# gongaa/Feedback-GNN

Measured on NVIDIA B200. Metric: decoded frames/sec (BP->GNN->BP, [[1270,28]]), higher is better.
Workload: dtype f32

## Files before the change

### feedback-gnn_b200/csrc/fbgnn_gbp_tc.cuh

```cuda
#ifndef FBGNN_GBP_TC_CUH
#define FBGNN_GBP_TC_CUH

#include "fbgnn_kernels.cuh"

namespace fbgnn {
namespace tc {

__device__ __forceinline__ uint32_t smem_u32(const void *p) { return (uint32_t)__cvta_generic_to_shared(p); }

__device__ __forceinline__ void tmem_alloc(uint32_t *slot, uint32_t ncols) {
    asm volatile("tcgen05.alloc.cta_group::1.sync.aligned.shared::cta.b32 [%0], %1;" :: "r"(smem_u32(slot)), "r"(ncols) : "memory");
    asm volatile("tcgen05.relinquish_alloc_permit.cta_group::1.sync.aligned;" ::: "memory");
}
__device__ __forceinline__ void tmem_dealloc(uint32_t taddr, uint32_t ncols) {
    asm volatile("tcgen05.dealloc.cta_group::1.sync.aligned.b32 %0, %1;" :: "r"(taddr), "r"(ncols) : "memory");
}
__device__ __forceinline__ void tc_fence_before() { asm volatile("tcgen05.fence::before_thread_sync;" ::: "memory"); }
__device__ __forceinline__ void tc_fence_after() { asm volatile("tcgen05.fence::after_thread_sync;" ::: "memory"); }
__device__ __forceinline__ void fence_async_smem() { asm volatile("fence.proxy.async.shared::cta;" ::: "memory"); }
__device__ __forceinline__ void tmem_wait_st() { asm volatile("tcgen05.wait::st.sync.aligned;" ::: "memory"); }
__device__ __forceinline__ void tmem_wait_ld() { asm volatile("tcgen05.wait::ld.sync.aligned;" ::: "memory"); }

__device__ __forceinline__ void tmem_st8(uint32_t taddr, const uint32_t v[8]) {
    asm volatile("tcgen05.st.sync.aligned.32x32b.x8.b32 [%0], {%1, %2, %3, %4, %5, %6, %7, %8};"
                 :: "r"(taddr), "r"(v[0]), "r"(v[1]), "r"(v[2]), "r"(v[3]), "r"(v[4]), "r"(v[5]), "r"(v[6]), "r"(v[7]) : "memory");
}
__device__ __forceinline__ void tmem_ld8(uint32_t taddr, float v[8]) {
    uint32_t r[8];
    asm volatile("tcgen05.ld.sync.aligned.32x32b.x8.b32 {%0, %1, %2, %3, %4, %5, %6, %7}, [%8];"
                 : "=r"(r[0]), "=r"(r[1]), "=r"(r[2]), "=r"(r[3]), "=r"(r[4]), "=r"(r[5]), "=r"(r[6]), "=r"(r[7]) : "r"(taddr) : "memory");
    asm volatile("tcgen05.wait::ld.sync.aligned;" ::: "memory");
#pragma unroll
    for (int q = 0; q < 8; q++) v[q] = __uint_as_float(r[q]);
}

__device__ __forceinline__ void umma_tf32_ts(uint32_t d_tmem, uint32_t a_tmem, uint64_t b_desc, uint32_t idesc, uint32_t accumulate) {
    asm volatile("{\n\t.reg .pred p;\n\tsetp.ne.b32 p, %4, 0;\n\t"
                 "tcgen05.mma.cta_group::1.kind::tf32 [%0], [%1], %2, %3, p;\n\t}"
                 :: "r"(d_tmem), "r"(a_tmem), "l"(b_desc), "r"(idesc), "r"(accumulate) : "memory");
}
__device__ __forceinline__ void umma_commit(uint32_t bar) {
    asm volatile("tcgen05.commit.cta_group::1.mbarrier::arrive::one.shared::cluster.b64 [%0];" :: "r"(bar) : "memory");
}
__device__ __forceinline__ void mbar_init(uint64_t *bar, uint32_t count) {
    asm volatile("mbarrier.init.shared::cta.b64 [%0], %1;" :: "r"(smem_u32(bar)), "r"(count) : "memory");
    asm volatile("fence.mbarrier_init.release.cluster;" ::: "memory");
}
__device__ __forceinline__ void mbar_wait(uint32_t bar, uint32_t parity) {
    uint32_t ok;
    do {
        asm volatile("{\n\t.reg .pred p;\n\tmbarrier.try_wait.parity.shared::cta.b64 p, [%1], %2;\n\tselp.b32 %0, 1, 0, p;\n\t}"
                     : "=r"(ok) : "r"(bar), "r"(parity) : "memory");
    } while (!ok);
}

__host__ __device__ inline int b_tile_offset(int n, int k, int kpad) {
    return (n >> 3) * (kpad / 4) * 32 + (k >> 2) * 32 + (n & 7) * 4 + (k & 3);
}
__device__ __forceinline__ uint64_t b_desc(uint32_t saddr, int kpad) {
    const uint64_t lbo = 128 >> 4, sbo = (uint64_t)((kpad / 4) * 128) >> 4;
    return (uint64_t)((saddr & 0x3FFFF) >> 4) | (lbo << 16) | (sbo << 32) | (1ull << 46);
}
__host__ __device__ inline uint32_t idesc_tf32(int npad) {
    return (1u << 4) | (2u << 7) | (2u << 10) | ((uint32_t)(npad >> 3) << 17) | ((128u >> 4) << 24);
}
__host__ __device__ inline float tf32_hi(float x) {
#ifdef __CUDA_ARCH__
    return __uint_as_float((__float_as_uint(x) + 0x1000u) & 0xffffe000u);
#else
    uint32_t u; memcpy(&u, &x, 4); u = (u + 0x1000u) & 0xffffe000u; float r; memcpy(&r, &u, 4); return r;
#endif
}

constexpr int t(int k, int n) { return 2 * k * n; }
struct VnW {
    static constexpr int B1X = 0, B1Z = B1X + t(24, 48);
    static constexpr int W2X = B1Z + t(24, 48), W2Z = W2X + t(40, 32);
    static constexpr int W3AB = W2Z + t(40, 32);
    static constexpr int W3C = W3AB + t(40, 48);
    static constexpr int W4 = W3C + t(24, 48);
    static constexpr int W5 = W4 + t(40, 32);
    static constexpr int BIAS = W5 + t(24, 80);
    static constexpr int total = BIAS + 180;
};
struct CnW {
    static constexpr int B1 = 0, W2 = B1 + t(24, 48);
    static constexpr int W3A = W2 + t(40, 32);
    static constexpr int W3B = W3A + t(24, 48);
    static constexpr int W4 = W3B + t(24, 48);
    static constexpr int W5 = W4 + t(40, 32);
    static constexpr int BIAS = W5 + t(24, 48);
    static constexpr int total = BIAS + 120;
};

struct Grp {
    uint32_t tmem;
    uint32_t lane_base;
    uint32_t bar;
    uint32_t phase;
    int gid;
    bool leader;
};

__device__ __forceinline__ void grp_sync(int gid) { asm volatile("bar.sync %0, 128;" :: "r"(gid + 1) : "memory"); }

template <int KPAD>
__device__ __forceinline__ void store_a(const Grp &g, int col_hi, int col_lo, const float *a) {
    __syncwarp();
#pragma unroll
    for (int k0 = 0; k0 < KPAD; k0 += 8) {
        uint32_t hi[8], lo[8];
#pragma unroll
        for (int q = 0; q < 8; q++) {
            const float h = tf32_hi(a[k0 + q]);
            hi[q] = __float_as_uint(h);
            lo[q] = __float_as_uint(a[k0 + q] - h);
        }
        tmem_st8(g.lane_base + col_hi + k0, hi);
        tmem_st8(g.lane_base + col_lo + k0, lo);
    }
}

__device__ __forceinline__ void gemm(Grp &g, int col_ahi, int col_alo, int kpad, int col_d, uint32_t b_saddr, int npad,
                                     bool accumulate) {
    __syncwarp();
    tmem_wait_st();
    tmem_wait_ld();
    tc_fence_before();
    grp_sync(g.gid);
    if (g.leader) {
        tc_fence_after();
        const uint32_t idesc = idesc_tf32(npad);
        const uint32_t bl = b_saddr + (uint32_t)(npad * kpad * 4);
        for (int s = 0; s < kpad / 8; s++) {
            const uint64_t dh = b_desc(b_saddr + s * 256, kpad), dl = b_desc(bl + s * 256, kpad);
            umma_tf32_ts(g.tmem + col_d, g.tmem + col_ahi + s * 8, dh, idesc, (accumulate || s > 0) ? 1u : 0u);
            umma_tf32_ts(g.tmem + col_d, g.tmem + col_alo + s * 8, dh, idesc, 1u);
            umma_tf32_ts(g.tmem + col_d, g.tmem + col_ahi + s * 8, dl, idesc, 1u);
        }
        umma_commit(g.bar);
    }
    mbar_wait(g.bar, g.phase);
    g.phase ^= 1u;
    tc_fence_after();
    __syncwarp();
}

template <typename MATH, typename SENDER>
__device__ __forceinline__ int recv_tc(const Grp &g, int col_base, const float *__restrict__ b1, int e0, int e1,
                                       const float *__restrict__ rows, int row_stride, uint32_t *codes, int cstride,
                                       SENDER sender) {
    constexpr int JB = 8, H = 40;
    gbp_stage_codes(codes, cstride, e0, e1, sender);
    auto code_at = [&](int e) -> uint32_t { return (e - e0 < GBP_CODE_CAP) ? codes[(e - e0) * cstride] : sender(e); };
    int ssum = 0;
    uint32_t c0 = 0;
    float4 nx0 = make_float4(0.0f, 0.0f, 0.0f, 0.0f), nx1 = nx0;
    if (e0 < e1) {
        c0 = code_at(e0);
        const float *pf = rows + (int64_t)(c0 >> 1) * row_stride;
        nx0 = *reinterpret_cast<const float4 *>(pf); nx1 = *reinterpret_cast<const float4 *>(pf + 4);
    }
#pragma unroll 1
    for (int j = 0; j < H; j += JB) {
        float bs[JB], hs[JB];
        __syncwarp();
        tmem_ld8(g.lane_base + col_base + j, bs);
        const float4 ba = *reinterpret_cast<const float4 *>(b1 + j), bb = *reinterpret_cast<const float4 *>(b1 + j + 4);
        bs[0] += ba.x; bs[1] += ba.y; bs[2] += ba.z; bs[3] += ba.w; bs[4] += bb.x; bs[5] += bb.y; bs[6] += bb.z; bs[7] += bb.w;
#pragma unroll
        for (int q = 0; q < JB; q++) hs[q] = 0.0f;
        uint32_t cc = c0;
#pragma unroll 1
        for (int e = e0; e < e1; e++) {
            const float pq[JB] = {nx0.x, nx0.y, nx0.z, nx0.w, nx1.x, nx1.y, nx1.z, nx1.w};
            const bool neg = (cc & 1u) != 0;
            if (e + 1 < e1) {
                cc = code_at(e + 1);
                const float *pf = rows + (int64_t)(cc >> 1) * row_stride + j;
                nx0 = *reinterpret_cast<const float4 *>(pf); nx1 = *reinterpret_cast<const float4 *>(pf + 4);
            }
            if (j == 0) ssum += neg ? -1 : 1;
#pragma unroll
            for (int q = 0; q < JB; q++) {
                float t = MATH::tanh(pq[q] + bs[q]);
                hs[q] += neg ? -t : t;
            }
        }
        if (j + JB < H && e0 < e1) {
            const float *pf = rows + (int64_t)(c0 >> 1) * row_stride + j + JB;
            nx0 = *reinterpret_cast<const float4 *>(pf); nx1 = *reinterpret_cast<const float4 *>(pf + 4);
        }
        uint32_t hi[JB], lo[JB];
#pragma unroll
        for (int q = 0; q < JB; q++) {
            const float h = tf32_hi(hs[q]);
            hi[q] = __float_as_uint(h);
            lo[q] = __float_as_uint(hs[q] - h);
        }
        __syncwarp();
        tmem_st8(g.lane_base + j, hi);
        tmem_st8(g.lane_base + H + j, lo);
    }
    return ssum;
}

__device__ __forceinline__ void bulk_g2s(uint32_t dst_saddr, const void *src, uint32_t bytes, uint32_t bar) {
    asm volatile("cp.async.bulk.shared::cluster.global.mbarrier::complete_tx::bytes [%0], [%1], %2, [%3];"
                 :: "r"(dst_saddr), "l"(src), "r"(bytes), "r"(bar) : "memory");
}
__device__ __forceinline__ void mbar_expect_tx(uint32_t bar, uint32_t bytes) {
    asm volatile("mbarrier.arrive.expect_tx.shared::cta.b64 _, [%0], %1;" :: "r"(bar), "r"(bytes) : "memory");
}

__device__ __forceinline__ Grp cta_setup(float *sm, const float *__restrict__ wsrc, int nfloats, uint64_t *bars, uint32_t *tslot) {
    __shared__ uint64_t load_bar;
    if (threadIdx.x < 32) tmem_alloc(tslot, 256);
    if (threadIdx.x == 32) {
        mbar_init(&bars[0], 1); mbar_init(&bars[1], 1); mbar_init(&load_bar, 1);
        fence_async_smem();
        const uint32_t bytes = (uint32_t)nfloats * 4u, bar = smem_u32(&load_bar), dst = smem_u32(sm);
        mbar_expect_tx(bar, bytes);
        constexpr uint32_t CHUNK = 32768;
        for (uint32_t off = 0; off < bytes; off += CHUNK)
            bulk_g2s(dst + off, reinterpret_cast<const char *>(wsrc) + off, min(CHUNK, bytes - off), bar);
    }
    tc_fence_before();
    __syncthreads();
    tc_fence_after();
    mbar_wait(smem_u32(&load_bar), 0);
    Grp g;
    g.gid = threadIdx.x >> 7;
    const int t = threadIdx.x & 127;
    g.tmem = *tslot + (uint32_t)(g.gid * 128);
    g.lane_base = g.tmem + ((uint32_t)((t >> 5) * 32) << 16);
    g.bar = smem_u32(&bars[g.gid]);
    g.phase = 0;
    g.leader = t == 0;
    return g;
}

__device__ __forceinline__ void cta_teardown(const uint32_t *tslot) {
    tmem_wait_ld();
    tmem_wait_st();
    tc_fence_before();
    __syncthreads();
    if (threadIdx.x < 32) tmem_dealloc(*tslot, 256);
}

template <typename MATH>
__global__ void __launch_bounds__(256, 2) k_gbp_vn_tc(const GbpArgs a, const float *__restrict__ wtc) {
    constexpr int D = 20, H = 40, M = 20;
    extern __shared__ __align__(128) float sm[];
    __shared__ uint64_t bars[2];
    __shared__ uint32_t tslot;
    Grp g = cta_setup(sm, wtc, VnW::total, bars, &tslot);
    const uint32_t sbase = smem_u32(sm);
    const float *bias = sm + VnW::BIAS;
    uint32_t *codes = reinterpret_cast<uint32_t *>(sm + VnW::total) + threadIdx.x;
    const int n = a.X.n, mt = a.X.m + a.Z.m, t = threadIdx.x & 127;
    const int64_t total = a.B * n, ntiles = (total + 127) / 128;
    for (int64_t tile = (int64_t)blockIdx.x * 2 + g.gid; tile < ntiles; tile += (int64_t)gridDim.x * 2) {
        const int64_t it = tile * 128 + t;
        const bool valid = it < total;
        const int64_t b = valid ? it / n : 0;
        const int v = valid ? (int)(it - b * n) : 0;
        float own[24], mm[2 * M];
#pragma unroll
        for (int k = 0; k < 24; k++) own[k] = 0.0f;
        if (valid) {
#pragma unroll
            for (int k = 0; k < D; k += 4) {
                const float4 v4 = *reinterpret_cast<const float4 *>(a.h_vn + it * D + k);
                own[k] = v4.x; own[k + 1] = v4.y; own[k + 2] = v4.z; own[k + 3] = v4.w;
            }
        }
#pragma unroll 1
        for (int side = 0; side < 2; side++) {
            const SideDev &S = side ? a.Z : a.X;
            const float *pf_b = a.pfc + (b * mt + (side ? a.X.m : 0)) * H;
            const uint8_t *sy = side ? a.sz + b * a.Z.m : a.sx + b * a.X.m;
            const idx_t *vn_cn = S.vn_cn;
            const int e0 = valid ? S.vn_ptr[v] : 0, e1 = valid ? S.vn_ptr[v + 1] : 0;
            store_a<24>(g, 0, 24, own);
            gemm(g, 0, 24, 24, 80, sbase + 4 * (side ? VnW::B1Z : VnW::B1X), 48, false);
            const int ssum = recv_tc<MATH>(g, 80, bias + side * H, e0, e1, pf_b, H, codes, 256,
                                           [&](int e) { const uint32_t c = vn_cn[e]; return (c << 1) | (sy[c] != 0 ? 1u : 0u); });
            gemm(g, 0, 40, 40, 80, sbase + 4 * (side ? VnW::W2Z : VnW::W2X), 32, false);
            const float fs = (float)ssum, dg = (float)(e1 - e0);
            const float *b2 = bias + 2 * H + side * M;
#pragma unroll
            for (int c0 = 0; c0 < 24; c0 += 8) {
                float d[8];
                tmem_ld8(g.lane_base + 80 + c0, d);
#pragma unroll
                for (int q = 0; q < 8; q++) {
                    if (c0 + q < M) {
                        float r = d[q] + fs * b2[c0 + q];
                        if (a.reduce == 0 && e1 > e0) r = r / dg;
                        if (side == 0) mm[c0 + q] = r;
                        else mm[M + c0 + q] = r;
                    }
                }
            }
        }
        store_a<40>(g, 0, 40, mm);
        gemm(g, 0, 40, 40, 80, sbase + 4 * VnW::W3AB, 48, false);
        store_a<24>(g, 0, 24, own);
        gemm(g, 0, 24, 24, 80, sbase + 4 * VnW::W3C, 48, true);
        float hid[H];
        const float *b3 = bias + 2 * H + 2 * M;
#pragma unroll
        for (int c0 = 0; c0 < H; c0 += 8) {
            float d[8];
            tmem_ld8(g.lane_base + 80 + c0, d);
#pragma unroll
            for (int q = 0; q < 8; q++) hid[c0 + q] = MATH::tanh(d[q] + b3[c0 + q]);
        }
        store_a<40>(g, 0, 40, hid);
        gemm(g, 0, 40, 40, 80, sbase + 4 * VnW::W4, 32, false);
        float out[24];
        const float *b4 = b3 + H;
#pragma unroll
        for (int c0 = 0; c0 < 24; c0 += 8) {
            float d[8];
            tmem_ld8(g.lane_base + 80 + c0, d);
#pragma unroll
            for (int q = 0; q < 8; q++) out[c0 + q] = (c0 + q < D) ? d[q] + b4[c0 + q] : 0.0f;
        }
        if (valid) {
#pragma unroll
            for (int k = 0; k < D; k += 4)
                *reinterpret_cast<float4 *>(a.h_vn + it * D + k) = make_float4(out[k], out[k + 1], out[k + 2], out[k + 3]);
        }
        store_a<24>(g, 80, 104, out);
        gemm(g, 80, 104, 24, 0, sbase + 4 * VnW::W5, 80, false);
#pragma unroll 1
        for (int c0 = 0; c0 < 2 * H; c0 += 8) {
            float d[8];
            __syncwarp();
            tmem_ld8(g.lane_base + c0, d);
            if (valid) {
                float *dst = a.pfv + it * 2 * H + c0;
                *reinterpret_cast<float4 *>(dst) = make_float4(d[0], d[1], d[2], d[3]);
                *reinterpret_cast<float4 *>(dst + 4) = make_float4(d[4], d[5], d[6], d[7]);
            }
        }
    }
    cta_teardown(&tslot);
}

template <typename MATH>
__global__ void __launch_bounds__(256, 2) k_gbp_cn_tc(const GbpArgs a, const float *__restrict__ wtc, int side) {
    constexpr int D = 20, H = 40, M = 20;
    extern __shared__ __align__(128) float sm[];
    __shared__ uint64_t bars[2];
    __shared__ uint32_t tslot;
    Grp g = cta_setup(sm, wtc, CnW::total, bars, &tslot);
    const uint32_t sbase = smem_u32(sm);
    const float *bias = sm + CnW::BIAS;
    uint32_t *codes = reinterpret_cast<uint32_t *>(sm + CnW::total) + threadIdx.x;
    const SideDev &S = side ? a.Z : a.X;
    const int n = a.X.n, mt = a.X.m + a.Z.m, ms = S.m, coff = side ? a.X.m : 0, t = threadIdx.x & 127;
    const idx_t *cn_vn = S.cn_vn;
    float *hcs = side ? a.hcz : a.hcx;
    const uint8_t *sys = side ? a.sz : a.sx;
    const int64_t total = a.B * ms, ntiles = (total + 127) / 128;
    for (int64_t tile = (int64_t)blockIdx.x * 2 + g.gid; tile < ntiles; tile += (int64_t)gridDim.x * 2) {
        const int64_t it = tile * 128 + t;
        const bool valid = it < total;
        const int64_t b = valid ? it / ms : 0;
        const int c = valid ? (int)(it - b * ms) : 0;
        float own[24], in[24];
#pragma unroll
        for (int k = 0; k < 24; k++) { own[k] = 0.0f; in[k] = 0.0f; }
        int e0 = 0, e1 = 0;
        if (valid) {
#pragma unroll
            for (int k = 0; k < D; k += 4) {
                const float4 v4 = *reinterpret_cast<const float4 *>(hcs + it * D + k);
                own[k] = v4.x; own[k + 1] = v4.y; own[k + 2] = v4.z; own[k + 3] = v4.w;
            }
            e0 = S.cn_ptr[c]; e1 = S.cn_ptr[c + 1];
            if (!a.zero_logits) {
                const float lgv = a.lg[b * mt + coff + c];
                in[M] = sys[it] ? -lgv : lgv;
            }
        }
        const float *pf_b = a.pfv + b * n * 2 * H + (side ? H : 0);
        store_a<24>(g, 0, 24, own);
        gemm(g, 0, 24, 24, 80, sbase + 4 * CnW::B1, 48, false);
        recv_tc<MATH>(g, 80, bias, e0, e1, pf_b, 2 * H, codes, 256, [&](int e) { return (uint32_t)cn_vn[e] << 1; });
        gemm(g, 0, 40, 40, 80, sbase + 4 * CnW::W2, 32, false);
        const float dg = (float)(e1 - e0);
        const float *b2 = bias + H;
#pragma unroll
        for (int c0 = 0; c0 < 24; c0 += 8) {
            float d[8];
            tmem_ld8(g.lane_base + 80 + c0, d);
#pragma unroll
            for (int q = 0; q < 8; q++) {
                if (c0 + q < M) {
                    float r = d[q] + dg * b2[c0 + q];
                    if (a.reduce == 0 && e1 > e0) r = r / dg;
                    in[c0 + q] = r;
                }
            }
        }
        store_a<24>(g, 0, 24, in);
        gemm(g, 0, 24, 24, 80, sbase + 4 * CnW::W3A, 48, false);
        store_a<24>(g, 0, 24, own);
        gemm(g, 0, 24, 24, 80, sbase + 4 * CnW::W3B, 48, true);
        float hid[H];
        const float *b3 = bias + H + M;
#pragma unroll
        for (int c0 = 0; c0 < H; c0 += 8) {
            float d[8];
            tmem_ld8(g.lane_base + 80 + c0, d);
#pragma unroll
            for (int q = 0; q < 8; q++) hid[c0 + q] = MATH::tanh(d[q] + b3[c0 + q]);
        }
        store_a<40>(g, 0, 40, hid);
        gemm(g, 0, 40, 40, 80, sbase + 4 * CnW::W4, 32, false);
        float out[24];
        const float *b4 = b3 + H;
#pragma unroll
        for (int c0 = 0; c0 < 24; c0 += 8) {
            float d[8];
            tmem_ld8(g.lane_base + 80 + c0, d);
#pragma unroll
            for (int q = 0; q < 8; q++) out[c0 + q] = (c0 + q < D) ? d[q] + b4[c0 + q] : 0.0f;
        }
        if (valid) {
#pragma unroll
            for (int k = 0; k < D; k += 4)
                *reinterpret_cast<float4 *>(hcs + it * D + k) = make_float4(out[k], out[k + 1], out[k + 2], out[k + 3]);
        }
        store_a<24>(g, 80, 104, out);
        gemm(g, 80, 104, 24, 0, sbase + 4 * CnW::W5, 48, false);
#pragma unroll 1
        for (int c0 = 0; c0 < H; c0 += 8) {
            float d[8];
            __syncwarp();
            tmem_ld8(g.lane_base + c0, d);
            if (valid) {
                float *dst = a.pfc + (b * mt + coff + c) * H + c0;
                *reinterpret_cast<float4 *>(dst) = make_float4(d[0], d[1], d[2], d[3]);
                *reinterpret_cast<float4 *>(dst + 4) = make_float4(d[4], d[5], d[6], d[7]);
            }
        }
    }
    cta_teardown(&tslot);
}

}
}

#endif
```

### feedback-gnn_b200/csrc/fbgnn_gnn_tc.cuh

```cuda
#ifndef FBGNN_GNN_TC_CUH
#define FBGNN_GNN_TC_CUH

#include "fbgnn_gbp_tc.cuh"

namespace fbgnn {
namespace tc {

struct GnnW {
    static constexpr int H = 40, M = 20;
    static constexpr int W2X = 0, W2Z = W2X + t(40, 32);
    static constexpr int W3AB = W2Z + t(40, 32);
    static constexpr int SCALAR = W3AB + t(40, 48);
    static constexpr int total = SCALAR + GnnLayout<40, 20>::total;
};

template <int DV, typename MATH>
__device__ __forceinline__ void gnn_edges_tc(const Grp &g, const float *__restrict__ w1p, const float *__restrict__ b1,
                                             const float hc[DV], float f1, float f2, float f3) {
    constexpr int H = 40, JB = 8;
#pragma unroll 1
    for (int j0 = 0; j0 < H; j0 += JB) {
        uint32_t hi[JB], lo[JB];
#pragma unroll
        for (int q = 0; q < JB; q += 2) {
            const float4 wa = *reinterpret_cast<const float4 *>(w1p + 4 * (j0 + q));
            const float4 wb = *reinterpret_cast<const float4 *>(w1p + 4 * (j0 + q) + 4);
            float2 hs;
            if constexpr (MATH::kPaired) {
                const float2 wcn = make_float2(wa.x, wa.y);
                const float2 base = FB_FMA2(fb2s(f3), make_float2(wb.z, wb.w), FB_FMA2(fb2s(f2), make_float2(wb.x, wb.y),
                                            FB_FMA2(fb2s(f1), make_float2(wa.z, wa.w), make_float2(b1[j0 + q], b1[j0 + q + 1]))));
                hs = MATH::tanh2(FB_FMA2(fb2s(hc[0]), wcn, base));
#pragma unroll
                for (int k = 1; k < DV; k++) hs = FB_ADD2(hs, MATH::tanh2(FB_FMA2(fb2s(hc[k]), wcn, base)));
            } else {
                const float base0 = FB_FMA(f3, wb.z, FB_FMA(f2, wb.x, FB_FMA(f1, wa.z, b1[j0 + q])));
                const float base1 = FB_FMA(f3, wb.w, FB_FMA(f2, wb.y, FB_FMA(f1, wa.w, b1[j0 + q + 1])));
                hs.x = MATH::tanh(FB_FMA(hc[0], wa.x, base0));
                hs.y = MATH::tanh(FB_FMA(hc[0], wa.y, base1));
#pragma unroll
                for (int k = 1; k < DV; k++) {
                    hs.x = FB_ADD(hs.x, MATH::tanh(FB_FMA(hc[k], wa.x, base0)));
                    hs.y = FB_ADD(hs.y, MATH::tanh(FB_FMA(hc[k], wa.y, base1)));
                }
            }
            const float2 h = make_float2(tf32_hi(hs.x), tf32_hi(hs.y));
            const float2 l = MATH::kPaired ? FB_SUB2(hs, h) : make_float2(FB_SUB(hs.x, h.x), FB_SUB(hs.y, h.y));
            hi[q] = __float_as_uint(h.x); hi[q + 1] = __float_as_uint(h.y);
            lo[q] = __float_as_uint(l.x); lo[q + 1] = __float_as_uint(l.y);
        }
        __syncwarp();
        tmem_st8(g.lane_base + j0, hi);
        tmem_st8(g.lane_base + H + j0, lo);
    }
}

template <int DV, typename MATH>
__global__ void __launch_bounds__(256, 2) k_gnn_tc(const GnnArgs a, const float *__restrict__ wtc) {
    constexpr int H = 40, M = 20;
    typedef GnnLayout<H, M> Lay;
    extern __shared__ __align__(128) float sm[];
    __shared__ uint64_t bars[2];
    __shared__ uint32_t tslot;
    Grp g = cta_setup(sm, wtc, GnnW::total, bars, &tslot);
    const uint32_t sbase = smem_u32(sm);
    const float *ws = sm + GnnW::SCALAR;
    const int n = a.X.n, t = threadIdx.x & 127;
    const int64_t total = a.num_frames * n, ntiles = (total + 127) / 128;
    const float dg = (float)DV;
    auto fetch = [&](int64_t tile, float &q1, float &q2, float &q3, float (&qx)[DV], float (&qz)[DV], int64_t &qb, int &qv) -> bool {
        const int64_t it = tile * 128 + t;
        const bool ok = tile < ntiles && it < total;
        q1 = q2 = q3 = 0.0f;
#pragma unroll
        for (int k = 0; k < DV; k++) { qx[k] = 0.0f; qz[k] = 0.0f; }
        qb = 0; qv = 0;
        if (ok) {
            const int64_t fi = it / n;
            qv = (int)(it - fi * n);
            qb = a.frame_list ? a.frame_list[fi] : fi;
            q1 = a.h_vn(qb, qv, 0); q2 = a.h_vn(qb, qv, 1); q3 = a.h_vn(qb, qv, 2);
#pragma unroll
            for (int k = 0; k < DV; k++) {
                const int cx = a.X.vn_cn[qv * DV + k], cz = a.Z.vn_cn[qv * DV + k];
                const float lx = a.logit_hx(cx, qb), lz = a.logit_hz(cz, qb);
                qx[k] = a.sx(cx, qb) ? -lx : lx;
                qz[k] = a.sz(cz, qb) ? -lz : lz;
            }
        }
        return ok;
    };
    float n1, n2, n3, nhx[DV], nhz[DV];
    int64_t nb;
    int nv;
    bool nvalid = fetch((int64_t)blockIdx.x * 2 + g.gid, n1, n2, n3, nhx, nhz, nb, nv);
    for (int64_t tile = (int64_t)blockIdx.x * 2 + g.gid; tile < ntiles; tile += (int64_t)gridDim.x * 2) {
        const bool valid = nvalid;
        const int64_t b = nb;
        const int v = nv;
        const float f1 = n1, f2 = n2, f3 = n3;
        float hcx[DV], hcz[DV];
#pragma unroll
        for (int k = 0; k < DV; k++) { hcx[k] = nhx[k]; hcz[k] = nhz[k]; }
        nvalid = fetch(tile + (int64_t)gridDim.x * 2, n1, n2, n3, nhx, nhz, nb, nv);
        float mm[2 * M];
#pragma unroll 1
        for (int side = 0; side < 2; side++) {
            gnn_edges_tc<DV, MATH>(g, ws + (side ? Lay::W1tz : Lay::W1tx), ws + (side ? Lay::b1z : Lay::b1x),
                                   side ? hcz : hcx, f1, f2, f3);
            gemm(g, 0, H, H, 80, sbase + 4 * (side ? GnnW::W2Z : GnnW::W2X), 32, false);
            const float *b2 = ws + (side ? Lay::b2z : Lay::b2x);
#pragma unroll
            for (int c0 = 0; c0 < 24; c0 += 8) {
                float d[8];
                tmem_ld8(g.lane_base + 80 + c0, d);
#pragma unroll
                for (int q = 0; q < 8; q++) {
                    if (c0 + q < M) {
                        const float r = (a.reduce == 0) ? FB_ADD(d[q], b2[c0 + q]) : FB_FMA(dg, b2[c0 + q], d[q]);
                        if (side == 0) mm[c0 + q] = r;
                        else mm[M + c0 + q] = r;
                    }
                }
            }
        }
        store_a<2 * M>(g, 0, 2 * M, mm);
        gemm(g, 0, 2 * M, 2 * M, 80, sbase + 4 * GnnW::W3AB, 48, false);
        float o0 = 0.0f, o1 = 0.0f, o2 = 0.0f;
#pragma unroll 1
        for (int c0 = 0; c0 < H; c0 += 8) {
            float d[8];
            tmem_ld8(g.lane_base + 80 + c0, d);
            if constexpr (MATH::kPaired) {
#pragma unroll
                for (int q = 0; q < 8; q += 2) {
                    const int j = c0 + q;
                    auto row = [&](int off) { return make_float2(ws[off + j], ws[off + j + 1]); };
                    float2 h = FB_FMA2(fb2s(f1), row(Lay::W3 + (2 * M) * H), make_float2(d[q], d[q + 1]));
                    h = FB_FMA2(fb2s(f2), row(Lay::W3 + (2 * M + 1) * H), h);
                    h = FB_FMA2(fb2s(f3), row(Lay::W3 + (2 * M + 2) * H), h);
                    h = MATH::tanh2(FB_ADD2(h, row(Lay::b3)));
                    o0 = FB_FMA(h.x, ws[Lay::W0 + j * 3 + 0], o0);
                    o1 = FB_FMA(h.x, ws[Lay::W0 + j * 3 + 1], o1);
                    o2 = FB_FMA(h.x, ws[Lay::W0 + j * 3 + 2], o2);
                    o0 = FB_FMA(h.y, ws[Lay::W0 + j * 3 + 3], o0);
                    o1 = FB_FMA(h.y, ws[Lay::W0 + j * 3 + 4], o1);
                    o2 = FB_FMA(h.y, ws[Lay::W0 + j * 3 + 5], o2);
                }
                continue;
            }
#pragma unroll
            for (int q = 0; q < 8; q++) {
                const int j = c0 + q;
                float h = FB_FMA(f1, ws[Lay::W3 + (2 * M) * H + j], d[q]);
                h = FB_FMA(f2, ws[Lay::W3 + (2 * M + 1) * H + j], h);
                h = FB_FMA(f3, ws[Lay::W3 + (2 * M + 2) * H + j], h);
                h = MATH::tanh(FB_ADD(h, ws[Lay::b3 + j]));
                o0 = FB_FMA(h, ws[Lay::W0 + j * 3 + 0], o0);
                o1 = FB_FMA(h, ws[Lay::W0 + j * 3 + 1], o1);
                o2 = FB_FMA(h, ws[Lay::W0 + j * 3 + 2], o2);
            }
        }
        if (valid) {
            a.out(b, v, 0) = FB_ADD(o0, ws[Lay::b0 + 0]);
            a.out(b, v, 1) = FB_ADD(o1, ws[Lay::b0 + 1]);
            a.out(b, v, 2) = FB_ADD(o2, ws[Lay::b0 + 2]);
        }
    }
    cta_teardown(&tslot);
}

static __global__ void __launch_bounds__(128) k_umma_probe(const float *A, const float *B, const float *Din, float *Dout,
                                                           int trials) {
    __shared__ __align__(128) float sb[128];
    __shared__ uint64_t bar;
    __shared__ uint32_t tslot;
    const int t = threadIdx.x, warp = t >> 5;
    if (warp == 0) tmem_alloc(&tslot, 32);
    if (t == 0) { mbar_init(&bar, 1); fence_async_smem(); }
    tc_fence_before();
    __syncthreads();
    tc_fence_after();
    const uint32_t tbase = tslot, lane_base = tbase + ((uint32_t)(warp * 32) << 16);
    for (int tr = 0; tr < trials; tr++) {
        sb[b_tile_offset(t >> 3, t & 7, 8)] = B[(tr * 8 + (t & 7)) * 16 + (t >> 3)];
        uint32_t a[8], d0[8], d1[8];
#pragma unroll
        for (int q = 0; q < 8; q++) {
            a[q] = __float_as_uint(A[((int64_t)tr * 128 + t) * 8 + q]);
            d0[q] = __float_as_uint(Din[((int64_t)tr * 128 + t) * 16 + q]);
            d1[q] = __float_as_uint(Din[((int64_t)tr * 128 + t) * 16 + 8 + q]);
        }
        tmem_st8(lane_base + 0, a);
        tmem_st8(lane_base + 16, d0);
        tmem_st8(lane_base + 24, d1);
        tmem_wait_st();
        fence_async_smem();
        tc_fence_before();
        __syncthreads();
        if (t == 0) {
            tc_fence_after();
            umma_tf32_ts(tbase + 16, tbase + 0, b_desc(smem_u32(sb), 8), idesc_tf32(16), 1u);
            umma_commit(smem_u32(&bar));
        }
        mbar_wait(smem_u32(&bar), (uint32_t)(tr & 1));
        tc_fence_after();
        float v[8];
        tmem_ld8(lane_base + 16, v);
#pragma unroll
        for (int q = 0; q < 8; q++) Dout[((int64_t)tr * 128 + t) * 16 + q] = v[q];
        tmem_ld8(lane_base + 24, v);
#pragma unroll
        for (int q = 0; q < 8; q++) Dout[((int64_t)tr * 128 + t) * 16 + 8 + q] = v[q];
        tc_fence_before();
        __syncthreads();
    }
    if (warp == 0) tmem_dealloc(tbase, 32);
}

}
}

#endif
```

Measured before the change: 467,800.

## Overlap X-side W2 tensor-core GEMM with first Z-side edge block compute

Splits the GEMM helper into separate issue and wait steps. In the GNN kernel, the X-side W2 MMA is now issued asynchronously, and the first 8-column block of Z-side edge tanh features is computed in registers while it runs. The kernel then waits, reads the X result out of TMEM, and stores the precomputed Z block into the A columns the GEMM just consumed. This hides some MMA latency behind SFU work, at the cost of extra live registers and more code.

```diff
diff --git a/feedback-gnn_b200/csrc/fbgnn_gbp_tc.cuh b/feedback-gnn_b200/csrc/fbgnn_gbp_tc.cuh
--- a/feedback-gnn_b200/csrc/fbgnn_gbp_tc.cuh
+++ b/feedback-gnn_b200/csrc/fbgnn_gbp_tc.cuh
@@ -121,8 +121,8 @@
     }
 }
 
-__device__ __forceinline__ void gemm(Grp &g, int col_ahi, int col_alo, int kpad, int col_d, uint32_t b_saddr, int npad,
-                                     bool accumulate) {
+__device__ __forceinline__ void gemm_issue(const Grp &g, int col_ahi, int col_alo, int kpad, int col_d, uint32_t b_saddr,
+                                           int npad, bool accumulate) {
     __syncwarp();
     tmem_wait_st();
     tmem_wait_ld();
@@ -140,10 +140,17 @@
         }
         umma_commit(g.bar);
     }
+}
+__device__ __forceinline__ void gemm_wait(Grp &g) {
     mbar_wait(g.bar, g.phase);
     g.phase ^= 1u;
     tc_fence_after();
     __syncwarp();
+}
+__device__ __forceinline__ void gemm(Grp &g, int col_ahi, int col_alo, int kpad, int col_d, uint32_t b_saddr, int npad,
+                                     bool accumulate) {
+    gemm_issue(g, col_ahi, col_alo, kpad, col_d, b_saddr, npad, accumulate);
+    gemm_wait(g);
 }
 
 template <typename MATH, typename SENDER>
diff --git a/feedback-gnn_b200/csrc/fbgnn_gnn_tc.cuh b/feedback-gnn_b200/csrc/fbgnn_gnn_tc.cuh
--- a/feedback-gnn_b200/csrc/fbgnn_gnn_tc.cuh
+++ b/feedback-gnn_b200/csrc/fbgnn_gnn_tc.cuh
@@ -15,40 +15,46 @@
 };
 
 template <int DV, typename MATH>
+__device__ __forceinline__ void gnn_edge_block(const float *__restrict__ w1p, const float *__restrict__ b1, const float hc[DV],
+                                               float f1, float f2, float f3, int j0, uint32_t hi[8], uint32_t lo[8]) {
+#pragma unroll
+    for (int q = 0; q < 8; q += 2) {
+        const float4 wa = *reinterpret_cast<const float4 *>(w1p + 4 * (j0 + q));
+        const float4 wb = *reinterpret_cast<const float4 *>(w1p + 4 * (j0 + q) + 4);
+        float2 hs;
+        if constexpr (MATH::kPaired) {
+            const float2 wcn = make_float2(wa.x, wa.y);
+            const float2 base = FB_FMA2(fb2s(f3), make_float2(wb.z, wb.w), FB_FMA2(fb2s(f2), make_float2(wb.x, wb.y),
+                                        FB_FMA2(fb2s(f1), make_float2(wa.z, wa.w), make_float2(b1[j0 + q], b1[j0 + q + 1]))));
+            hs = MATH::tanh2(FB_FMA2(fb2s(hc[0]), wcn, base));
+#pragma unroll
+            for (int k = 1; k < DV; k++) hs = FB_ADD2(hs, MATH::tanh2(FB_FMA2(fb2s(hc[k]), wcn, base)));
+        } else {
+            const float base0 = FB_FMA(f3, wb.z, FB_FMA(f2, wb.x, FB_FMA(f1, wa.z, b1[j0 + q])));
+            const float base1 = FB_FMA(f3, wb.w, FB_FMA(f2, wb.y, FB_FMA(f1, wa.w, b1[j0 + q + 1])));
+            hs.x = MATH::tanh(FB_FMA(hc[0], wa.x, base0));
+            hs.y = MATH::tanh(FB_FMA(hc[0], wa.y, base1));
+#pragma unroll
+            for (int k = 1; k < DV; k++) {
+                hs.x = FB_ADD(hs.x, MATH::tanh(FB_FMA(hc[k], wa.x, base0)));
+                hs.y = FB_ADD(hs.y, MATH::tanh(FB_FMA(hc[k], wa.y, base1)));
+            }
+        }
+        const float2 h = make_float2(tf32_hi(hs.x), tf32_hi(hs.y));
+        const float2 l = MATH::kPaired ? FB_SUB2(hs, h) : make_float2(FB_SUB(hs.x, h.x), FB_SUB(hs.y, h.y));
+        hi[q] = __float_as_uint(h.x); hi[q + 1] = __float_as_uint(h.y);
+        lo[q] = __float_as_uint(l.x); lo[q + 1] = __float_as_uint(l.y);
+    }
+}
+
+template <int DV, typename MATH>
 __device__ __forceinline__ void gnn_edges_tc(const Grp &g, const float *__restrict__ w1p, const float *__restrict__ b1,
-                                             const float hc[DV], float f1, float f2, float f3) {
+                                             const float hc[DV], float f1, float f2, float f3, int j_first) {
     constexpr int H = 40, JB = 8;
 #pragma unroll 1
-    for (int j0 = 0; j0 < H; j0 += JB) {
+    for (int j0 = j_first; j0 < H; j0 += JB) {
         uint32_t hi[JB], lo[JB];
-#pragma unroll
-        for (int q = 0; q < JB; q += 2) {
-            const float4 wa = *reinterpret_cast<const float4 *>(w1p + 4 * (j0 + q));
-            const float4 wb = *reinterpret_cast<const float4 *>(w1p + 4 * (j0 + q) + 4);
-            float2 hs;
-            if constexpr (MATH::kPaired) {
-                const float2 wcn = make_float2(wa.x, wa.y);
-                const float2 base = FB_FMA2(fb2s(f3), make_float2(wb.z, wb.w), FB_FMA2(fb2s(f2), make_float2(wb.x, wb.y),
-                                            FB_FMA2(fb2s(f1), make_float2(wa.z, wa.w), make_float2(b1[j0 + q], b1[j0 + q + 1]))));
-                hs = MATH::tanh2(FB_FMA2(fb2s(hc[0]), wcn, base));
-#pragma unroll
-                for (int k = 1; k < DV; k++) hs = FB_ADD2(hs, MATH::tanh2(FB_FMA2(fb2s(hc[k]), wcn, base)));
-            } else {
-                const float base0 = FB_FMA(f3, wb.z, FB_FMA(f2, wb.x, FB_FMA(f1, wa.z, b1[j0 + q])));
-                const float base1 = FB_FMA(f3, wb.w, FB_FMA(f2, wb.y, FB_FMA(f1, wa.w, b1[j0 + q + 1])));
-                hs.x = MATH::tanh(FB_FMA(hc[0], wa.x, base0));
-                hs.y = MATH::tanh(FB_FMA(hc[0], wa.y, base1));
-#pragma unroll
-                for (int k = 1; k < DV; k++) {
-                    hs.x = FB_ADD(hs.x, MATH::tanh(FB_FMA(hc[k], wa.x, base0)));
-                    hs.y = FB_ADD(hs.y, MATH::tanh(FB_FMA(hc[k], wa.y, base1)));
-                }
-            }
-            const float2 h = make_float2(tf32_hi(hs.x), tf32_hi(hs.y));
-            const float2 l = MATH::kPaired ? FB_SUB2(hs, h) : make_float2(FB_SUB(hs.x, h.x), FB_SUB(hs.y, h.y));
-            hi[q] = __float_as_uint(h.x); hi[q + 1] = __float_as_uint(h.y);
-            lo[q] = __float_as_uint(l.x); lo[q + 1] = __float_as_uint(l.y);
-        }
+        gnn_edge_block<DV, MATH>(w1p, b1, hc, f1, f2, f3, j0, hi, lo);
         __syncwarp();
         tmem_st8(g.lane_base + j0, hi);
         tmem_st8(g.lane_base + H + j0, lo);
@@ -104,26 +110,30 @@
         for (int k = 0; k < DV; k++) { hcx[k] = nhx[k]; hcz[k] = nhz[k]; }
         nvalid = fetch(tile + (int64_t)gridDim.x * 2, n1, n2, n3, nhx, nhz, nb, nv);
         float mm[2 * M];
-#pragma unroll 1
-        for (int side = 0; side < 2; side++) {
-            gnn_edges_tc<DV, MATH>(g, ws + (side ? Lay::W1tz : Lay::W1tx), ws + (side ? Lay::b1z : Lay::b1x),
-                                   side ? hcz : hcx, f1, f2, f3);
-            gemm(g, 0, H, H, 80, sbase + 4 * (side ? GnnW::W2Z : GnnW::W2X), 32, false);
-            const float *b2 = ws + (side ? Lay::b2z : Lay::b2x);
+        auto w2_out = [&](const float *b2, float *out) {
 #pragma unroll
             for (int c0 = 0; c0 < 24; c0 += 8) {
                 float d[8];
                 tmem_ld8(g.lane_base + 80 + c0, d);
 #pragma unroll
-                for (int q = 0; q < 8; q++) {
-                    if (c0 + q < M) {
-                        const float r = (a.reduce == 0) ? FB_ADD(d[q], b2[c0 + q]) : FB_FMA(dg, b2[c0 + q], d[q]);
-                        if (side == 0) mm[c0 + q] = r;
-                        else mm[M + c0 + q] = r;
-                    }
-                }
-            }
-        }
+                for (int q = 0; q < 8; q++)
+                    if (c0 + q < M) out[c0 + q] = (a.reduce == 0) ? FB_ADD(d[q], b2[c0 + q]) : FB_FMA(dg, b2[c0 + q], d[q]);
+            }
+        };
+        gnn_edges_tc<DV, MATH>(g, ws + Lay::W1tx, ws + Lay::b1x, hcx, f1, f2, f3, 0);
+        gemm_issue(g, 0, H, H, 80, sbase + 4 * GnnW::W2X, 32, false);
+        {
+            uint32_t hi[8], lo[8];
+            gnn_edge_block<DV, MATH>(ws + Lay::W1tz, ws + Lay::b1z, hcz, f1, f2, f3, 0, hi, lo);
+            gemm_wait(g);
+            w2_out(ws + Lay::b2x, mm);
+            __syncwarp();
+            tmem_st8(g.lane_base + 0, hi);
+            tmem_st8(g.lane_base + H, lo);
+        }
+        gnn_edges_tc<DV, MATH>(g, ws + Lay::W1tz, ws + Lay::b1z, hcz, f1, f2, f3, 8);
+        gemm(g, 0, H, H, 80, sbase + 4 * GnnW::W2Z, 32, false);
+        w2_out(ws + Lay::b2z, mm + M);
         store_a<2 * M>(g, 0, 2 * M, mm);
         gemm(g, 0, 2 * M, 2 * M, 80, sbase + 4 * GnnW::W3AB, 48, false);
         float o0 = 0.0f, o1 = 0.0f, o2 = 0.0f;
```

After: 478,800, median of 6. +2.3%, better.
